# maotian123/loc_lib

Measured on AMD Instinct MI355X. Metric: scans/sec (64x1800-pt scan vs 10M-pt map) + ICP iter ms, higher is better.
Workload: dtype f64; 1 GPU; BASELINE configs[2]: 256 scans/GPU x 115200 pts (64x1800, cityblock-v1) vs one 10000000-pt map, P2PLANE ICP, reference defaults (alpha=0.1 KD-tree ANN, eps=1e-2, max 20 iters), scans sharded by rank, no collective; includes scan H2D: every step aligns a batch copied host->HBM for it (pinned double buffer, copy stream, overlapped with the previous step); 3 alignment(s) in flight; scans_per_gpu=256, map_points=10000000, pipeline_depth=3, search_mode=tree_faithful_ann, tree_depth=30, tree_bytes=239999992

## Files before the change

### loc_lib_amd/api.py

```python
import ctypes
import os
import subprocess

import numpy as np

_HERE = os.path.dirname(os.path.abspath(__file__))
LIB_PATH = os.environ.get("LOCGPU_LIB") or os.path.join(_HERE, "liblocgpu.so")
CSRC = os.path.join(_HERE, "csrc")

P2P, P2LINE, P2PLANE = 0, 1, 2
P2PLANE_MAP = 5
SEARCH_TREE_FAITHFUL, SEARCH_GRID_EXACT = 0, 1
CENTER, NEARBY6 = 0, 1
DIRECT_NDT, INCREMENTAL_NDT = 1, 2

ABI_SYMBOLS = [
    "locgpu_icp_opts_default", "locgpu_ndt_opts_default", "locgpu_create", "locgpu_destroy", "locgpu_last_error",
    "locgpu_device_count", "locgpu_icp_set_target", "locgpu_icp_set_target_async", "locgpu_icp_target_info", "locgpu_knn", "locgpu_icp_hb", "locgpu_icp_align",
    "locgpu_transform_cloud", "locgpu_batch_create", "locgpu_batch_destroy", "locgpu_icp_align_batch", "locgpu_ndt_align_batch",
    "locgpu_icp_hb_batch", "locgpu_gn_update", "locgpu_ndt_set_target", "locgpu_ndt_target_info", "locgpu_ndt_dump",
    "locgpu_ndt_align", "locgpu_profile_enable", "locgpu_profile_read", "locgpu_visit_count_enable", "locgpu_visit_count_read",
    "locgpu_search_stats_read", "locgpu_debug_batch_nn", "locgpu_graph_enable",
    "locgpu_cloud_create", "locgpu_cloud_destroy", "locgpu_cloud_upload", "locgpu_cloud_info", "locgpu_cloud_download", "locgpu_cloud_copy",
    "locgpu_cloud_remove_nan", "locgpu_cloud_voxel_filter", "locgpu_cloud_crop_box", "locgpu_cloud_transform", "locgpu_cloud_append",
# ... 591 lines not shown
        out = np.zeros(6)
        self._check(lib().locgpu_profile_read(self._h, out.ctypes.data, int(reset)))
        return dict(search_ms=out[0], accum_ms=out[1], solve_ms=out[2], search_n=int(out[3]), accum_n=int(out[4]), solve_n=int(out[5]))

    def visit_count_enable(self, on=True):
        self._check(lib().locgpu_visit_count_enable(self._h, int(on)))

    def visit_count_read(self, reset=True):
        out = np.zeros(4, dtype=np.uint64)
        self._check(lib().locgpu_visit_count_read(self._h, out.ctypes.data, int(reset)))
        return dict(nodes=int(out[0]), leaves=int(out[1]), queries=int(out[2]), distinct_slots=int(out[3]))


    def debug_batch_nn(self, batch, k=5):
        out = np.empty((batch.n_local, batch.max_points, k), dtype=np.int32)
        self._check(lib().locgpu_debug_batch_nn(self._h, batch._h, int(k), out.ctypes.data))
        return out

    def search_stats_read(self, reset=True):
        out = np.zeros(4, dtype=np.uint64)
        self._check(lib().locgpu_search_stats_read(self._h, out.ctypes.data, int(reset)))
        return dict(searched=int(out[0]), redone=int(out[1]), walked=int(out[2]), replayed=int(out[3]))


def _xyzi(a):
    a = np.ascontiguousarray(a, dtype=np.float32)
    if a.ndim != 2 or a.shape[1] != 4:
        raise ValueError("cloud must be [n, 4] float32 (x, y, z, intensity)")
    return a


class Cloud:

    def __init__(self, ctx, points=None, is_dense=True, _borrowed=None):
        self.ctx = ctx
        self._owned = _borrowed is None
        if _borrowed is not None:
            self._h = _borrowed
        else:
            self._h = ctypes.c_void_p()
            ctx._check(lib().locgpu_cloud_create(ctx._h, ctypes.byref(self._h)))
            if points is not None:
                self.upload(points, is_dense)

    def upload(self, points, is_dense=True):
        a = _xyzi(points)
# ... 429 lines not shown
```

### loc_lib_amd/csrc/context.hpp

```cpp
#pragma once
#include <hip/hip_runtime.h>

#include <string>
#include <vector>

#include "../../include/locgpu.h"
#include "batch_upload.hpp"
#include "device_math.hpp"
#include "grid_kernels.hpp"
#include "icp_kernels.hpp"

#include "host_worker.hpp"

struct NdtTable;
namespace locgpu { struct IncNdtState; struct FilterScratch; }

namespace locgpu {
struct PendingTarget;
struct AlignSpec {
    GnParams prm{};
    float alpha = 1.0f;
    bool grid = false;
    bool ndt() const { return method_is_ndt(prm.method); }
    int k() const { return method_k(prm.method); }
// ... 78 lines not shown
    int slot = 0;
    hipStream_t stream = nullptr;
    int n_scans = 0, max_n = 0, blocks_per_scan = 0;
    int n_total = 0, first = 0;
    bool sharded = false;
    double* d_acc = nullptr;
    size_t pitch = 0;
    float4* d_src = nullptr;
    int* d_counts = nullptr;
    locgpu::PoseState* d_state = nullptr;
    uint32_t* d_nn = nullptr;
    bool shared_src = false;
    int* d_src_of = nullptr;
    int cap_scans = 0, split_scans = 0;
    size_t cap_points = 0;
    const float4* d_src_ext = nullptr;
    bool counters_clean = false;
    int last_iterations = -1;
    double* d_partials = nullptr;
    double* d_hb = nullptr;
    uint32_t* d_redo_list = nullptr;
    unsigned int* d_redo_count = nullptr;
    uint32_t* d_redo_list2 = nullptr;
    uint32_t* d_grid_qkey = nullptr;
    uint2* d_grid_sorted = nullptr;
    uint32_t* d_grid_tile_count = nullptr;
    void* d_grid_scan_temp = nullptr;
    size_t grid_tocc_cap = 0, grid_scan_cap = 0;
    hipGraphExec_t graph_exec = nullptr;
    hipGraphExec_t graph_exec_next = nullptr;
    locgpu::AlignSpec graph_spec;
    const void* graph_target = nullptr;
    unsigned long long graph_epoch = 0;
    float4* h_src = nullptr;
    hipEvent_t xyz_ev[8] = {};
    locgpu::PoseState* h_state = nullptr;
    unsigned long long* h_post = nullptr;
    static constexpr int kPostWord = 16;
    unsigned int post_call = 0;
    bool paced_tail = false;
    hipEvent_t tail_ev = nullptr;
    double* h_hb = nullptr;
    int* h_active = nullptr;
    int* d_active = nullptr;
    std::vector<int> counts;
    locgpu::BatchUploadState upl;
// ... 39 lines not shown
```

### loc_lib_amd/csrc/gn_driver.hip

```cpp
#include <algorithm>
#include <chrono>
#include <cmath>
#include <cstdlib>
#include <cstring>
#include <string>
#include <thread>

#include "batch_upload.hpp"
#include "env.hpp"
#include "gn_driver.hpp"
#include "ndt_inc.hpp"
#include "ndt_kernels.hpp"

namespace locgpu {

namespace {
inline int next_chunk(const locgpu_batch* b) { return b->n_total == 1 ? 2 : kNextChunk; }
inline int first_chunk_len(const locgpu_batch* b) {
    if (b->n_total != 1 || b->sharded || b->last_iterations < 0) return kFirstChunk;
    return std::min(kLongFirstChunk, std::max(3, b->last_iterations + 1));
}

}

SearchArgs make_search_args(const locgpu_ctx* ctx, const locgpu_batch* b, const float4* src, const PoseState* st, int k, float alpha_eff, bool skip_nonfinite) {
    SearchArgs sa{ctx->d_tree, ctx->tree_slots * sizeof(uint64_t), ctx->depth, src, b->d_counts, st, b->d_nn, b->pitch, b->max_n, b->n_scans, k, alpha_eff,
                  skip_nonfinite ? 1 : 0, nullptr, b->d_redo_list, b->d_redo_count, b->d_redo_list2, b->d_redo_count + 1, ctx->d_search_stats};
    if (!ctx->tree_bounded) sa.redo_list = nullptr;
    return sa;
}

void init_state(PoseState& ps, const double pose[7]) {
    std::memset(&ps, 0, sizeof(ps));
    for (int i = 0; i < 4; ++i) ps.q[i] = pose[i];
    for (int i = 0; i < 3; ++i) ps.t[i] = pose[4 + i];
    quat_to_R(ps.q, ps.R);
}

static void init_states(locgpu_batch* b, const double* poses) {
    for (int s = 0; s < b->n_total; ++s) init_state(b->h_state[s], poses + 7 * (size_t)s);
}

void write_scan_result(const PoseState& ps, const double* init, double* out_pose, locgpu_align_stats* stats) {
    if (ps.status == 1) {
        for (int j = 0; j < 7; ++j) out_pose[j] = init[j];
    } else {
        for (int j = 0; j < 4; ++j) out_pose[j] = ps.q[j];
        for (int j = 0; j < 3; ++j) out_pose[4 + j] = ps.t[j];
    }
    if (!stats) return;
// ... 494 lines not shown
```

### loc_lib_amd/csrc/icp_search.hip

```cpp
#include "env.hpp"
#include "icp_kernels.hpp"
#include "launch.hpp"
#include "search_walk.hpp"

#include <algorithm>
#include <iterator>
#include <type_traits>
#include <utility>

namespace locgpu {

template <int KMAX, int D, bool COUNT>
__global__ __launch_bounds__(kBlock) void icp_search_kernel(const uint2* __restrict__ tree, const float4* __restrict__ src,
                                                            const int* __restrict__ counts, const PoseState* __restrict__ st,
                                                            uint32_t* __restrict__ nn, size_t nn_pitch, int max_n, int k, float alpha_eff,
                                                            int skip_nonfinite, unsigned long long* __restrict__ visit_totals, uint32_t* __restrict__ touched,
                                                            const int* __restrict__ active, const int* __restrict__ src_of) {
    __shared__ uint32_t s_far[D][kBlock];
    __shared__ float s_d2[D][kBlock];
    const int scan = active ? active[blockIdx.y] : (int)blockIdx.y;
    if (st[scan].done) return;
    const int tid = threadIdx.x;
    const int i = blockIdx.x * kBlock + tid;
    if (i >= counts[scan]) return;
// ... 149 lines not shown
    for (unsigned int r0 = blockIdx.x * per_wave; r0 < n; r0 += gridDim.x * per_wave) {
        const unsigned int r = r0 + (unsigned int)tid;
        const bool valid = (unsigned int)tid < per_wave && r < n;
        const uint32_t gi = valid ? list[r] : 0u;
        Walk<K> w;
        w.qx = w.qy = w.qz = 0.f;
        if (valid) {
            int scan;
            const float4 p = list_point(src, src_of, max_n, gi, scan);
            const D3 qs = se3_apply(st[scan].q, st[scan].t, D3{(double)p.x, (double)p.y, (double)p.z});
            w.qx = (float)qs.x; w.qy = (float)qs.y; w.qz = (float)qs.z;
        }
        walk_query<K, ROWB>(rsrc, tree, w, valid, alpha_eff, 0, dummy, (uint32_t)(size_t)(&s_dyn[tid]), 0x7fffffff);
        const bool slow = valid && w.slow != 0u;
        if (valid && !slow) {
#pragma unroll
            for (int j = 0; j < K; ++j) nn[(size_t)j * nn_pitch + gi] = w.id[j];
        }
        if (!walk_exact_in_wave<K>(tree, slow, w.qx, w.qy, w.qz, alpha_eff, s_dyn, nn, nn_pitch, gi, search_stats))
            wave_append(redo_list, redo_count, slow, gi);
    }
}

constexpr int kRedoWaves = 2048;
constexpr int kDeepLanes = 64, kDeepWaves = 2048;
template <int KMAX, int D>
__global__ __launch_bounds__(64) void icp_search_redo_kernel(const uint2* __restrict__ tree, const float4* __restrict__ src,
                                                             const PoseState* __restrict__ st, uint32_t* __restrict__ nn, size_t nn_pitch,
                                                             int max_n, int k, float alpha_eff, const uint32_t* __restrict__ redo_list,
                                                             const unsigned int* __restrict__ redo_count, unsigned long long* __restrict__ search_stats,
                                                             const int* __restrict__ src_of) {
    __shared__ uint32_t s_far[D][64];
    __shared__ float s_d2[D][64];
    const unsigned int n = *redo_count;
    const int tid = threadIdx.x;
    if (blockIdx.x == 0 && tid == 0 && search_stats) atomicAdd(&search_stats[1], (unsigned long long)n);
    const unsigned int per_wave = min(64u, (n + gridDim.x - 1) / gridDim.x);
    if ((unsigned)tid >= per_wave) return;
    for (unsigned int r = blockIdx.x * per_wave + tid; r < n; r += gridDim.x * per_wave) {
        const size_t gi = redo_list[r];
        int scan;
        const float4 p = list_point(src, src_of, max_n, gi, scan);
        const D3 qs = se3_apply(st[scan].q, st[scan].t, D3{(double)p.x, (double)p.y, (double)p.z});
        KnnHeap<KMAX> heap;
        uint32_t nvis = 0, lvis = 0, out[KMAX];
        int cnt;
// ... 17 lines not shown
    KnnHeap<KMAX> heap;
    uint32_t nvis = 0, lvis = 0;
    tree_knn<KMAX, D, true>(tree, queries[3 * i], queries[3 * i + 1], queries[3 * i + 2], k, alpha_eff, s_far, s_d2, tid, heap, nvis, lvis);
    uint32_t out[KMAX];
    int cnt;
    heap_to_sorted<KMAX>(heap, out, cnt);
#pragma unroll
    for (int j = 0; j < KMAX; ++j)
        if (j < k) out_idx[i * k + j] = (out[j] == kInvalidSlot) ? -1 : (int32_t)(tree[out[j]].y & 0x3FFFFFFFu);
    if (visits) { visits[2 * i] = nvis; visits[2 * i + 1] = lvis; }
}

__global__ __launch_bounds__(kBlock) void count_touched_kernel(uint32_t* __restrict__ touched, size_t n_words, unsigned long long* __restrict__ totals) {
    unsigned long long c = 0;
    for (size_t i = (size_t)blockIdx.x * kBlock + threadIdx.x; i < n_words; i += (size_t)gridDim.x * kBlock) {
        c += (unsigned long long)__popc(touched[i]);
        touched[i] = 0u;
    }
    for (int off = 32; off > 0; off >>= 1) c += __shfl_xor(c, off, 64);
    if ((threadIdx.x & 63) == 0 && c) atomicAdd(&totals[3], c);
}

__global__ __launch_bounds__(kBlock) void nn_to_index_kernel(const uint2* __restrict__ tree, const uint32_t* __restrict__ nn, size_t nn_pitch, size_t n_queries,
                                                             int k, int32_t* __restrict__ out) {
    const size_t gi = (size_t)blockIdx.x * kBlock + threadIdx.x;
    if (gi >= n_queries) return;
    for (int j = 0; j < k; ++j) {
        const uint32_t slot = nn[(size_t)j * nn_pitch + gi];
        out[gi * k + j] = slot == kInvalidSlot ? -1 : (int32_t)(tree[slot].y & 0x3FFFFFFFu);
    }
}


template <class F>
static bool with_depth(int depth, F&& f) {
    if (depth <= 32) f(std::integral_constant<int, 32>{});
    else if (depth <= 40) f(std::integral_constant<int, 40>{});
    else if (depth <= 64) f(std::integral_constant<int, 64>{});
    else return false;
    return true;
}
template <bool UP_TO, class F>
static bool with_k(int k, F&& f) {
    if (k == 1) return f(std::integral_constant<int, 1>{});
    if (UP_TO ? k <= 5 : k == 5) return f(std::integral_constant<int, 5>{});
    if constexpr (UP_TO)
        if (k <= 8) return f(std::integral_constant<int, 8>{});
    return false;
}

bool stamp_build() {
    static const bool on = env_int("LOCGPU_STAMP", 0) != 0;
    return on;
}

void launch_nn_to_index(const uint2* tree, const uint32_t* nn, size_t nn_pitch, size_t n_queries, int k, int32_t* out, hipStream_t s) {
    hipLaunchKernelGGL(nn_to_index_kernel, dim3((unsigned)((n_queries + kBlock - 1) / kBlock)), dim3(kBlock), 0, s, tree, nn, nn_pitch, n_queries, k, out);
}

void launch_count_touched(uint32_t* touched, size_t n_words, unsigned long long* totals, hipStream_t s) {
    hipLaunchKernelGGL(count_touched_kernel, dim3(1024), dim3(kBlock), 0, s, touched, n_words, totals);
}

template <int KMAX, int D, bool COUNT>
static void launch_exact(const SearchArgs& a, hipStream_t s) {
    dim3 grid((a.max_n + kBlock - 1) / kBlock, a.active ? a.n_active : a.n_scans);
    hipLaunchKernelGGL((icp_search_kernel<KMAX, D, COUNT>), grid, dim3(kBlock), 0, s, a.tree, a.src, a.counts, a.st, a.nn, a.nn_pitch, a.max_n,
                       a.k, a.alpha_eff, a.skip_nonfinite, a.visit_totals, COUNT ? a.touched : nullptr, a.active, a.src_of);
}

struct WalkShape { int df, win; };
constexpr WalkShape kWalkShapes[] = {{10, 8}, {12, 0}, {15, 0}, {24, 0}};
template <class F, size_t... I>
static bool all_walk_shapes(F&& f, std::index_sequence<I...>) {
    return (f(std::integral_constant<int, kWalkShapes[I].df>{}, std::integral_constant<int, kWalkShapes[I].win>{}) && ...);
}
template <class F>
static bool all_walk_shapes(F&& f) { return all_walk_shapes(f, std::make_index_sequence<std::size(kWalkShapes)>{}); }

static int fast_stack_depth() {
    static const int v = [] {
        const int e = env_int("LOCGPU_FAST_STACK", kWalkShapes[0].df);
        for (const WalkShape& w : kWalkShapes)
            if (w.df == e) return e;
        return kWalkShapes[0].df;
    }();
    return v;
}
constexpr int kWindowStored = 13;

template <auto Kernel>
static bool no_static_lds() {
    hipFuncAttributes attr{};
    return hipFuncGetAttributes(&attr, reinterpret_cast<const void*>(Kernel)) == hipSuccess && attr.sharedSizeBytes == 0;
}
template <int K>
static bool walk_kernels_ok() {
    bool ok = all_walk_shapes([](auto DF, auto WIN) {
        return no_static_lds<icp_search_walk_kernel<K, DF(), 64, false, WIN()>>() && no_static_lds<icp_search_walk_kernel<K, DF(), 64, true, WIN()>>();
    });
    for (int depth : {32, 40, 64})
        with_depth(depth, [&](auto D) { ok = ok && no_static_lds<icp_search_walk_kernel<K, D() + 2, 16>>() && no_static_lds<icp_search_walk_list_kernel<K, D(), kDeepLanes>>(); });
    return ok;
}
bool search_kernels_lds_ok() {
    static const bool ok = walk_kernels_ok<1>() && walk_kernels_ok<5>();
    return ok;
}

template <int K, int D>
static void launch_redo(const SearchArgs& a, hipStream_t s) {
    hipLaunchKernelGGL((icp_search_redo_kernel<K, D>), dim3(kRedoWaves), dim3(64), 0, s, a.tree, a.src, a.st, a.nn, a.nn_pitch, a.max_n, a.k,
                       a.alpha_eff, a.redo_list, a.redo_count, a.search_stats, a.src_of);
}
template <int K, int D>
static void launch_walk_list(const SearchArgs& a, const uint32_t* list, const unsigned int* n_list, hipStream_t s) {
    hipLaunchKernelGGL((icp_search_walk_list_kernel<K, D, kDeepLanes>), dim3(kDeepWaves), dim3(64), (D + 2) * kDeepLanes * 8, s, a.tree, a.src, a.st, a.nn, a.nn_pitch, a.max_n,
                       a.alpha_eff, (unsigned int)a.tree_bytes + 16u, (uint32_t)(a.tree_bytes / 8), list, n_list, a.redo_list, a.redo_count, a.search_stats, a.src_of);
}

template <int K, int D, int DF, int WIN>
static void launch_walk(const SearchArgs& a, hipStream_t s) {
    const bool stamp = stamp_build();
    const uint32_t dummy = (uint32_t)(a.tree_bytes / 8);
    const unsigned int rsrc_bytes = (unsigned int)a.tree_bytes + 16u;
    const int n_launch = a.active ? a.n_active : a.n_scans;
    if (!stamp && (size_t)((a.max_n + 63) / 64) * n_launch <= 2048) {
        dim3 g1((a.max_n + 15) / 16, n_launch);
        hipLaunchKernelGGL((icp_search_walk_kernel<K, D + 2, 16>), g1, dim3(64), (D + 2) * 16 * 8, s, a.tree, a.src, a.counts, a.st, a.nn, a.nn_pitch, a.max_n,
                           a.alpha_eff, 0, rsrc_bytes, dummy, a.skip_nonfinite, a.redo_list, a.redo_count, a.redo_list2, a.redo_count2, a.search_stats, a.active, a.src_of);
        return;
    }
    const int stored = WIN ? kWindowStored : DF - 2;
    const int Tw = a.depth > stored ? a.depth - stored : 0;
    dim3 g2((a.max_n + 63) / 64, n_launch);
    static const bool lds_knob = env_flag("LOCGPU_K1_LDS_BYTES");
    unsigned lds_bytes = DF * 64 * 8;
    if (lds_knob) lds_bytes = (unsigned)std::max(env_int("LOCGPU_K1_LDS_BYTES", 0), DF * 64 * 8);
    if (stamp)
// ... 52 lines not shown
```

### loc_lib_amd/csrc/launch.hpp

```cpp
#pragma once
#include "gn_post.hpp"
#include <hip/hip_runtime.h>
#include <stdint.h>

#include "device_math.hpp"

namespace locgpu {

struct GnParams;

struct SearchArgs {
    const uint2* tree;
    size_t tree_bytes;
    int depth;
    const float4* src;
    const int* counts;
    const PoseState* st;
    uint32_t* nn;
    size_t nn_pitch;
    int max_n, n_scans, k;
    float alpha_eff;
    int skip_nonfinite;
    unsigned long long* visit_totals;
    uint32_t* redo_list;
    unsigned int* redo_count;
    uint32_t* redo_list2;
    unsigned int* redo_count2;
    unsigned long long* search_stats;
    const int* active = nullptr;
    int n_active = 0;
    const int* src_of = nullptr;
    uint32_t* touched = nullptr;
};

struct AccumArgs {
    const uint2* tree;
    const float4* src;
    const int* counts;
    const PoseState* st;
    const uint32_t* nn;
    size_t nn_pitch;
    int max_n, n_scans;
    double gate;
    double* partials;
    const int* active = nullptr;
    int n_active = 0;
    const int* src_of = nullptr;
    int split_scans = 0;
    const double* planes = nullptr;
};

bool launch_icp_search(const SearchArgs& a, hipStream_t s);
bool launch_icp_search_redo(const SearchArgs& a, hipStream_t s);
bool launch_icp_search_list(const SearchArgs& a, const uint32_t* list, const unsigned int* n_list, hipStream_t s);
bool launch_knn_query(const uint2* tree, int depth, const float* q, size_t nq, int k, float alpha_eff, int32_t* out, uint32_t* visits,
                      hipStream_t s);
// ... 27 lines not shown
    int max_n, n_scans;
    float gate2;
    double* partials;
    double* out;
    unsigned int* list_counts;
    const int* src_of = nullptr;
};
int icp_fitness_rows(int max_n);
void launch_icp_fitness(const FitnessArgs& a, hipStream_t s);
int launch_icp_fitness_accum(const FitnessArgs& a, hipStream_t s);
void launch_loam_fitness_sum(const double* const partials[2], const int rows[2], int n_cands, double* out, unsigned int* const list_counts[2], hipStream_t s);
void launch_fitness_sum(const double* partials, int rows, int n_scans, double* out, unsigned int* list_counts, hipStream_t s);
struct M12f { float v[12]; };
void launch_transform_cloud(const float4* src, size_t n, const M12f& m12, float* dst_xyz, hipStream_t s);
void launch_loam_join_transform(const float4* edge, size_t n_edge, const float4* surf, size_t n_surf, const M12f& m12, float4* out, hipStream_t s);
void launch_map_plane_queries(const uint2* tree, const uint32_t* leaf_slots, size_t first, int n, float4* src, int* counts, hipStream_t s);
void launch_map_plane_fit(const uint2* tree, const uint32_t* leaf_slots, size_t first, int n, const uint32_t* nn, size_t nn_pitch, double* planes,
                          unsigned long long* n_valid, hipStream_t s);
void launch_map_plane_dump(const uint2* tree, const uint32_t* leaf_slots, size_t n_leaves, const double* planes, size_t n_points, double* out_n4,
                           unsigned char* out_valid, hipStream_t s);
bool search_kernels_lds_ok();
bool stamp_build();
void launch_count_touched(uint32_t* touched, size_t n_words, unsigned long long* totals, hipStream_t s);
void launch_nn_to_index(const uint2* tree, const uint32_t* nn, size_t nn_pitch, size_t n_queries, int k, int32_t* out, hipStream_t s);

}
```

### loc_lib_amd/csrc/locgpu_api.hip

```cpp
#include <algorithm>
#include <atomic>
#include <cmath>
#include <cstdio>
#include <cstdlib>
#include <cstring>
#include <string>
#include <vector>

#include "batch_upload.hpp"
#include "cloud_filters.hpp"
#include "context.hpp"
#include "gn_driver.hpp"
#include "launch.hpp"
#include "ndt_inc.hpp"
#include "ndt_kernels.hpp"
#include "search_chunks.hpp"

using namespace locgpu;

namespace {
std::string g_create_err;
}

namespace locgpu {
// ... 10 lines not shown
}

static bool fill_now(locgpu_ctx* ctx, void* p, size_t bytes, const char* what) {
    return hip_ok(ctx, hipMemsetAsync(p, 0, bytes, ctx->stream), what) && hip_ok(ctx, hipStreamSynchronize(ctx->stream), what);
}

void locgpu::free_batch(locgpu_batch* b) {
    if (!b) return;
    upload_free_batch(b);
    for (hipEvent_t ev : b->stage_ev.ev) (void)hipEventDestroy(ev);
    if (b->ev_ready) (void)hipEventDestroy(b->ev_ready);
    if (b->ev_reduced) (void)hipEventDestroy(b->ev_reduced);
    if (b->d_src) (void)hipFree(b->d_src);
    if (b->d_src_of) (void)hipFree(b->d_src_of);
    if (b->d_counts) (void)hipFree(b->d_counts);
    if (b->d_state) (void)hipFree(b->d_state);
    if (b->d_nn) (void)hipFree(b->d_nn);
    if (b->d_partials) (void)hipFree(b->d_partials);
    if (b->d_hb) (void)hipFree(b->d_hb);
    if (b->d_acc) (void)hipFree(b->d_acc);
    if (b->d_redo_list) (void)hipFree(b->d_redo_list);
    if (b->d_redo_count) (void)hipFree(b->d_redo_count);
    if (b->d_redo_list2) (void)hipFree(b->d_redo_list2);
    if (b->d_grid_qkey) (void)hipFree(b->d_grid_qkey);
    if (b->d_grid_sorted) (void)hipFree(b->d_grid_sorted);
    if (b->d_grid_tile_count) (void)hipFree(b->d_grid_tile_count);
    if (b->d_grid_scan_temp) (void)hipFree(b->d_grid_scan_temp);
    if (b->graph_exec) (void)hipGraphExecDestroy(b->graph_exec);
    if (b->graph_exec_next) (void)hipGraphExecDestroy(b->graph_exec_next);
    if (b->h_src) (void)hipHostFree(b->h_src);
    if (b->h_state) (void)hipHostFree(b->h_state);
    if (b->h_post) (void)hipHostFree(b->h_post);
    if (b->tail_ev) (void)hipEventDestroy(b->tail_ev);
    for (hipEvent_t e : b->xyz_ev)
        if (e) (void)hipEventDestroy(e);
    if (b->h_hb) (void)hipHostFree(b->h_hb);
    if (b->h_active) (void)hipHostFree(b->h_active);
    if (b->d_active) (void)hipFree(b->d_active);
    delete b;
}

extern "C" {

void locgpu_icp_opts_default(locgpu_icp_opts* o) {
    if (!o) return;
    o->method = LOCGPU_P2P;
// ... 165 lines not shown
    if (n_scans < 0 || (n_scans == 0 && !sharded) || first < 0 || first + n_scans > n_total) return fail(ctx, LOCGPU_ERR_INVALID, "batch_create: bad arguments");
    if (n_total > 65535) return fail(ctx, LOCGPU_ERR_INVALID, "batch_create: at most 65535 scans per batch");
    if (n_scans > 65535) return fail(ctx, LOCGPU_ERR_INVALID, "batch_create: at most 65535 scans per batch");
    LOCGPU_HIP(ctx, hipSetDevice(ctx->device));
    if (n_scans == 0) max_n = 1;
    if (max_n == 0 || max_n > 0x7FFFFF00u || (size_t)n_scans * max_n > 0xFFFFFFF0ull)
        return fail(ctx, LOCGPU_ERR_INVALID, "batch_create: scans are empty or the batch exceeds 2^32 points");
    auto* b = new locgpu_batch();
    b->ctx = ctx;
    b->slot = ctx->next_slot;
    ctx->next_slot = (ctx->next_slot + 1) % locgpu_ctx::kSlots;
    b->stream = ctx->slot_stream[b->slot];
    b->n_scans = n_scans;
    b->n_total = n_total;
    b->first = first;
    b->sharded = sharded;
    b->max_n = (int)max_n;
    b->blocks_per_scan = (int)((max_n + kBlock - 1) / kBlock);
    b->pitch = (size_t)n_scans * max_n;
    b->counts.assign(n_scans, 0);
    b->shared_src = shared_src;
    b->cap_scans = n_scans;
    b->cap_points = max_n;
    bool ok = hip_ok(ctx, hipMalloc((void**)&b->d_src, std::max<size_t>(shared_src ? max_n : b->pitch, 1) * sizeof(float4)), "hipMalloc src") &&
              (!shared_src || (hip_ok(ctx, hipMalloc((void**)&b->d_src_of, (size_t)n_scans * sizeof(int)), "hipMalloc src_of") &&
                               fill_now(ctx, b->d_src_of, (size_t)n_scans * sizeof(int), "hipMemset src_of"))) &&
              hip_ok(ctx, hipMalloc((void**)&b->d_counts, std::max(n_scans, 1) * sizeof(int)), "hipMalloc counts") &&
              hip_ok(ctx, hipMalloc((void**)&b->d_state, n_total * sizeof(PoseState)), "hipMalloc state") &&
              (!sharded || hip_ok(ctx, hipMalloc((void**)&b->d_acc, (size_t)kFirstChunk * n_total * kAccW * sizeof(double)), "hipMalloc acc")) &&
              hip_ok(ctx, hipMalloc((void**)&b->d_nn, 5 * std::max<size_t>(b->pitch, 1) * sizeof(uint32_t)), "hipMalloc nn") &&
              hip_ok(ctx, hipMalloc((void**)&b->d_partials, (size_t)std::max(n_scans, 1) * b->blocks_per_scan * kAccW * sizeof(double)), "hipMalloc partials") &&
              hip_ok(ctx, hipMalloc((void**)&b->d_hb, (size_t)n_total * 44 * sizeof(double)), "hipMalloc hb") &&
              hip_ok(ctx, hipMalloc((void**)&b->d_redo_list, (stamp_build() ? 2 : 1) * std::max<size_t>(b->pitch, 1) * sizeof(uint32_t)), "hipMalloc redo") &&
              hip_ok(ctx, hipMalloc((void**)&b->d_redo_list2, std::max<size_t>(b->pitch, 1) * sizeof(uint32_t)), "hipMalloc redo2") &&
              hip_ok(ctx, hipMalloc((void**)&b->d_redo_count, 4 * sizeof(unsigned int)), "hipMalloc redo") &&
              hip_ok(ctx, hipHostMalloc((void**)&b->h_state, n_total * sizeof(PoseState)), "hipHostMalloc state") &&
              hip_ok(ctx, hipHostMalloc((void**)&b->h_hb, (size_t)n_total * 44 * sizeof(double)), "hipHostMalloc hb") &&
              hip_ok(ctx, hipHostMalloc((void**)&b->h_active, (size_t)std::max(n_scans, 1) * sizeof(int)), "hipHostMalloc active") &&
              hip_ok(ctx, hipMalloc((void**)&b->d_active, (size_t)std::max(n_scans, 1) * sizeof(int)), "hipMalloc active") &&
              fill_now(ctx, b->d_counts, std::max(n_scans, 1) * sizeof(int), "hipMemset counts") &&
              fill_now(ctx, b->d_redo_count, 4 * sizeof(unsigned int), "hipMemset redo");
    if (!ok) { free_batch(b); return LOCGPU_ERR_OOM; }
    *out = b;
    return LOCGPU_OK;
}

extern "C" {

static int make_batch(locgpu_ctx* ctx, const void* const* srcs, const size_t* counts, size_t stride_bytes, int n_scans, locgpu_batch** out,
                      int first = 0, int n_total = -1) {
    if (!ctx || !out) return LOCGPU_ERR_INVALID;
    *out = nullptr;
    if (n_scans < 0 || (n_scans > 0 && (!srcs || !counts)) || stride_bytes < 12) return fail(ctx, LOCGPU_ERR_INVALID, "batch_create: bad arguments");
    size_t max_n = 0;
    for (int s = 0; s < n_scans; ++s) max_n = std::max(max_n, counts[s]);
    for (int s = 0; s < n_scans; ++s)
        if (!srcs[s] && counts[s]) return fail(ctx, LOCGPU_ERR_INVALID, "batch_create: NULL scan pointer");
    locgpu_batch* b = nullptr;
// ... 182 lines not shown

int locgpu_icp_align(locgpu_ctx* ctx, const void* src, size_t n, size_t stride_bytes, const double init_pose[7], const locgpu_icp_opts* opts,
                     double out_pose[7], locgpu_align_stats* stats) {
    AlignSpec spec;
    const int rc = check_icp(ctx, opts, spec);
    return rc != LOCGPU_OK ? rc : align_single(ctx, spec, "icp_align", src && init_pose && out_pose, src, n, stride_bytes, nullptr, init_pose, out_pose, stats);
}

int locgpu_icp_hb_batch(locgpu_ctx* ctx, locgpu_batch* b, const double* poses, const locgpu_icp_opts* opts, double* hb) {
    AlignSpec spec;
    int rc = check_icp(ctx, opts, spec);
    if (rc == LOCGPU_OK) rc = check_batch(ctx, b, poses && hb, spec, "icp_hb_batch");
    return rc != LOCGPU_OK ? rc : eval_hb_batch(ctx, b, poses, spec, hb, "icp_hb_batch");
}

int locgpu_debug_batch_nn(locgpu_ctx* ctx, locgpu_batch* b, int k, int32_t* out) {
    if (!ctx || !b || b->ctx != ctx || !out || k < 1 || k > 5) return fail(ctx, LOCGPU_ERR_INVALID, "debug_batch_nn: bad arguments");
    { const int jrc = target_join(ctx); if (jrc != LOCGPU_OK) return jrc; }
    if (!ctx->d_tree) return fail(ctx, LOCGPU_ERR_NO_TARGET, "debug_batch_nn: no ICP target");
    LOCGPU_HIP(ctx, hipSetDevice(ctx->device));
    const size_t nq = (size_t)b->n_scans * b->max_n;
    int32_t* d_out = nullptr;
    LOCGPU_HIP(ctx, hipMalloc((void**)&d_out, nq * k * sizeof(int32_t)));
    launch_nn_to_index(ctx->d_tree, b->d_nn, b->pitch, nq, k, d_out, b->stream);
    const hipError_t e = hipMemcpyAsync(out, d_out, nq * k * sizeof(int32_t), hipMemcpyDeviceToHost, b->stream);
    const hipError_t e2 = hipStreamSynchronize(b->stream);
    (void)hipFree(d_out);
    LOCGPU_HIP(ctx, e);
    LOCGPU_HIP(ctx, e2);
    return LOCGPU_OK;
}

int locgpu_icp_hb(locgpu_ctx* ctx, const void* src, size_t n, size_t stride_bytes, const double pose[7], const locgpu_icp_opts* opts, double H[36],
                  double B[6], int64_t* effective_num, int* ok) {
    AlignSpec spec;
    int rc = check_icp(ctx, opts, spec);
    if (rc != LOCGPU_OK) return rc;
    if (!src || !pose || !H || !B) return fail(ctx, LOCGPU_ERR_INVALID, "icp_hb: bad arguments");
    locgpu_batch* b = nullptr;
    rc = single_batch(ctx, src, n, stride_bytes, &b);
    if (rc != LOCGPU_OK) return rc;
    double hb[44];
    rc = eval_hb_batch(ctx, b, pose, spec, hb, "icp_hb");
    if (rc != LOCGPU_OK) return rc;
    std::memcpy(H, hb, 36 * sizeof(double));
    std::memcpy(B, hb + 36, 6 * sizeof(double));
    if (effective_num) *effective_num = (int64_t)hb[42];
// ... 489 lines not shown
int locgpu_visit_count_read(locgpu_ctx* ctx, uint64_t out[4], int reset) {
    if (!ctx || !out) return LOCGPU_ERR_INVALID;
    out[0] = out[1] = out[2] = out[3] = 0;
    if (!ctx->d_visits) return LOCGPU_OK;
    LOCGPU_HIP(ctx, hipSetDevice(ctx->device));
    for (hipStream_t st : ctx->slot_stream) LOCGPU_HIP(ctx, hipStreamSynchronize(st));
    unsigned long long h[4];
    LOCGPU_HIP(ctx, hipMemcpy(h, ctx->d_visits, sizeof(h), hipMemcpyDeviceToHost));
    out[0] = h[0]; out[1] = h[1]; out[2] = h[2]; out[3] = h[3];
    if (reset && !fill_now(ctx, ctx->d_visits, sizeof(h), "hipMemset visits")) return LOCGPU_ERR_NO_DEVICE;
    return LOCGPU_OK;
}

}

extern "C" __attribute__((visibility("default"))) int locgpu_debug_stamp_trips(locgpu_ctx* ctx, locgpu_batch* b, uint32_t* out) {
    if (!ctx || !b || !out || !stamp_build()) return LOCGPU_ERR_INVALID;
    LOCGPU_HIP(ctx, hipSetDevice(ctx->device));
    LOCGPU_HIP(ctx, hipStreamSynchronize(b->stream));
    LOCGPU_HIP(ctx, hipMemcpy(out, b->d_redo_list + b->pitch, b->pitch * sizeof(uint32_t), hipMemcpyDeviceToHost));
    return LOCGPU_OK;
}

extern "C" __attribute__((visibility("default"))) size_t locgpu_debug_grid_dump(locgpu_ctx* ctx, int64_t info[9], float params[6], float* pts, size_t pts_cap,
                                                                                 void* tiles, size_t tiles_cap_bytes, uint32_t* hash, size_t hash_cap) {
    if (!ctx || target_join(ctx) != LOCGPU_OK || !ctx->d_tree || ensure_grid(ctx) != LOCGPU_OK) return 0;
    const locgpu::GridView& g = ctx->grid;
    if (info) {
        for (int a = 0; a < 3; ++a) { info[a] = g.dims[a]; info[6 + a] = g.tdims[a]; }
        info[3] = (int64_t)g.num_cells; info[4] = g.n_tocc; info[5] = (int64_t)g.tile_mask + 1;
    }
    if (params) { for (int a = 0; a < 3; ++a) params[a] = g.origin[a]; params[3] = g.cell; params[4] = g.inv_cell; params[5] = g.slack; }
    if (pts && hipMemcpy(pts, g.pts, std::min(pts_cap, g.num_points * 4) * sizeof(float), hipMemcpyDeviceToHost) != hipSuccess) return 0;
    if (tiles && hipMemcpy(tiles, g.tiles, std::min(tiles_cap_bytes, (size_t)g.n_tocc * sizeof(locgpu::TileRec)), hipMemcpyDeviceToHost) != hipSuccess) return 0;
    if (hash && hipMemcpy(hash, g.tile_hash, std::min(hash_cap, ((size_t)g.tile_mask + 1) * 2) * sizeof(uint32_t), hipMemcpyDeviceToHost) != hipSuccess) return 0;
    return g.num_points;
}

namespace locgpu {
void ndt_free(locgpu_ctx* ctx) {
    if (ctx->ndt) { ndt_table_free(*ctx->ndt); delete ctx->ndt; ctx->ndt = nullptr; }
    if (ctx->inc) { inc_ndt_destroy(ctx->inc); ctx->inc = nullptr; }
}
int check_ndt(locgpu_ctx* ctx, AlignSpec& spec) {
    if (!ctx) return LOCGPU_ERR_INVALID;
    const bool inc = ctx->ndt_opts.method == kNdtOptIncremental;
// ... 168 lines not shown
```

### loc_lib_amd/csrc/search_walk.hpp

```cpp
#pragma once
#include "icp_kernels.hpp"

namespace locgpu {

constexpr float kSentinelCoord = 3.0e38f;

template <int K>
struct Walk {
    float qx, qy, qz;
    float d[K];
    uint32_t id[K];
    uint32_t cur;
    int avail;
    uint32_t c3n;
    uint32_t slow;
    uint32_t rounds, wave_rounds;
};

typedef uint32_t __attribute__((address_space(3))) lds_u32;
typedef uint32_t u32x2 __attribute__((ext_vector_type(2)));
typedef u32x2 __attribute__((address_space(3))) lds_u32x2;

__device__ __forceinline__ lds_u32* lds_ptr(uint32_t byte_addr) { return reinterpret_cast<lds_u32*>(byte_addr); }

// ... 205 lines not shown
        for (int step = 0; step < C; ++step) {
            if (n.y < 0xC0000000u) {
                const uint32_t meta = n.y;
                const float th = as_f32(n.x);
                const float qa = meta < 0x40000000u ? qx : (meta < 0x80000000u ? qy : qz);
                const float dd = qa - th;
                const uint32_t nd2 = __float_as_uint(-(dd * dd));
                const uint32_t right = meta & 0x3FFFFFFFu;
                const bool go_left = qa < th;
                const uint32_t cur1 = cur + 1u;
                *reinterpret_cast<lds_u32x2*>(col_addr + (uint32_t)avail * ROWB) = u32x2{go_left ? right : cur1, nd2};
                avail += (int)nd2 < nbound ? 1 : 0;
                cur = go_left ? cur1 : right;
                n = __builtin_amdgcn_raw_buffer_load_b128(rsrc, (int)(cur << 3), 0, 0);
            }
        }
    } while (__ballot(cur != dummy || avail > 0) != 0ull);
#pragma unroll
    for (int j = 0; j < K; ++j) { w.d[j] = d[j]; w.id[j] = id[j]; }
    w.slow = slow; w.c3n = c3n; w.cur = cur; w.avail = avail;
    if (STAMP) { w.rounds = my_rounds; w.wave_rounds = all_rounds; }
}

}
```

Measured before the change: 12090 scans/s.

## Add spill-to-global ring-buffer stack for deep KD-tree list walks

Adds a new deep-query search kernel whose traversal stack is a small LDS ring window (default 8 rows) that spills older entries to a per-wave global buffer and reloads them in chunks when needed. This replaces the deep-list kernel that reserved a full depth-sized LDS stack per lane. The smaller LDS footprint allows higher occupancy, with waves_per_eu pinned at 8. The cost is extra global traffic and divergence on spill and reload, plus a fallback to the slow path when the spill rows overflow. It also masks nn_to_index output for padded query slots and adds a debug stats entry point.

```diff
diff --git a/loc_lib_amd/api.py b/loc_lib_amd/api.py
--- a/loc_lib_amd/api.py
+++ b/loc_lib_amd/api.py
@@ -637,6 +637,13 @@
         self._check(lib().locgpu_search_stats_read(self._h, out.ctypes.data, int(reset)))
         return dict(searched=int(out[0]), redone=int(out[1]), walked=int(out[2]), replayed=int(out[3]))
 
+    def debug_deep_stats(self):
+        fn = lib().locgpu_debug_deep_stats
+        fn.restype, fn.argtypes = ctypes.c_int, [ctypes.c_void_p, ctypes.c_void_p]
+        out = np.zeros(3, dtype=np.uint64)
+        self._check(fn(self._h, out.ctypes.data))
+        return dict(deep=int(out[0]), spilled=int(out[1]), reloaded=int(out[2]))
+
 
 def _xyzi(a):
     a = np.ascontiguousarray(a, dtype=np.float32)
diff --git a/loc_lib_amd/csrc/context.hpp b/loc_lib_amd/csrc/context.hpp
--- a/loc_lib_amd/csrc/context.hpp
+++ b/loc_lib_amd/csrc/context.hpp
@@ -124,6 +124,8 @@
     uint32_t* d_redo_list = nullptr;
     unsigned int* d_redo_count = nullptr;
     uint32_t* d_redo_list2 = nullptr;
+    uint2* d_deep_spill = nullptr;
+    int deep_spill_waves = 0;
     uint32_t* d_grid_qkey = nullptr;
     uint2* d_grid_sorted = nullptr;
     uint32_t* d_grid_tile_count = nullptr;
diff --git a/loc_lib_amd/csrc/gn_driver.hip b/loc_lib_amd/csrc/gn_driver.hip
--- a/loc_lib_amd/csrc/gn_driver.hip
+++ b/loc_lib_amd/csrc/gn_driver.hip
@@ -26,6 +26,7 @@
 SearchArgs make_search_args(const locgpu_ctx* ctx, const locgpu_batch* b, const float4* src, const PoseState* st, int k, float alpha_eff, bool skip_nonfinite) {
     SearchArgs sa{ctx->d_tree, ctx->tree_slots * sizeof(uint64_t), ctx->depth, src, b->d_counts, st, b->d_nn, b->pitch, b->max_n, b->n_scans, k, alpha_eff,
                   skip_nonfinite ? 1 : 0, nullptr, b->d_redo_list, b->d_redo_count, b->d_redo_list2, b->d_redo_count + 1, ctx->d_search_stats};
+    sa.deep_spill = b->d_deep_spill; sa.deep_spill_waves = b->deep_spill_waves;
     if (!ctx->tree_bounded) sa.redo_list = nullptr;
     return sa;
 }
diff --git a/loc_lib_amd/csrc/icp_search.hip b/loc_lib_amd/csrc/icp_search.hip
--- a/loc_lib_amd/csrc/icp_search.hip
+++ b/loc_lib_amd/csrc/icp_search.hip
@@ -195,6 +195,55 @@
     }
 }
 
+template <int K, int WIN, bool STAMP = false>
+__global__ __launch_bounds__(64) __attribute__((amdgpu_waves_per_eu(8, 8))) void icp_search_walk_spill_kernel(const uint2* __restrict__ tree, const float4* __restrict__ src,
+                                                                   const PoseState* __restrict__ st, uint32_t* __restrict__ nn, size_t nn_pitch, int max_n,
+                                                                   float alpha_eff, unsigned int tree_bytes, uint32_t dummy, const uint32_t* __restrict__ list,
+                                                                   const unsigned int* __restrict__ n_list, uint32_t* __restrict__ redo_list,
+                                                                   unsigned int* __restrict__ redo_count, unsigned long long* __restrict__ search_stats,
+                                                                   const int* __restrict__ src_of, uint2* __restrict__ spill, int spill_rows) {
+    extern __shared__ uint2 s_dyn[];
+    static_assert(WIN * 64 * 8 >= 64 * 2 * 8, "exact stack columns do not fit");
+    const unsigned int n = *n_list;
+    const int tid = threadIdx.x;
+    if (blockIdx.x == 0 && tid == 0 && search_stats) atomicAdd(&search_stats[2], (unsigned long long)n);
+    const __amdgpu_buffer_rsrc_t rsrc = __builtin_amdgcn_make_buffer_rsrc((void*)tree, 0, (int)tree_bytes, 0x00020000);
+    u32x2* spill_col = reinterpret_cast<u32x2*>(spill) + (size_t)blockIdx.x * (size_t)spill_rows * 64 + tid;
+    const unsigned int per_wave = min(64u, max(1u, (n + gridDim.x - 1) / gridDim.x));
+    for (unsigned int r0 = blockIdx.x * per_wave; r0 < n; r0 += gridDim.x * per_wave) {
+        const unsigned int r = r0 + (unsigned int)tid;
+        const bool valid = (unsigned int)tid < per_wave && r < n;
+        const uint32_t gi = valid ? list[r] : 0u;
+        Walk<K> w;
+        w.qx = w.qy = w.qz = 0.f;
+        if (valid) {
+            int scan;
+            const float4 p = list_point(src, src_of, max_n, gi, scan);
+            const D3 qs = se3_apply(st[scan].q, st[scan].t, D3{(double)p.x, (double)p.y, (double)p.z});
+            w.qx = (float)qs.x; w.qy = (float)qs.y; w.qz = (float)qs.z;
+        }
+#pragma unroll
+        for (int j = 0; j < K; ++j) { w.d[j] = __builtin_inff(); w.id[j] = kInvalidSlot; }
+        const bool sane = fabsf(w.qx) < 1e18f && fabsf(w.qy) < 1e18f && fabsf(w.qz) < 1e18f;
+        w.slow = valid && !sane ? 1u : 0u;
+        uint32_t n_spilled = 0, n_reloaded = 0;
+        walk_spill<K, WIN, LOCGPU_K1_C, STAMP>(rsrc, w, valid && sane, alpha_eff, dummy, (uint32_t)(size_t)(&s_dyn[tid]), spill_col, spill_rows, n_spilled, n_reloaded);
+#pragma unroll
+        for (int j = 0; j + 1 < K; ++j) w.slow |= w.d[j] == w.d[j + 1] ? 1u : 0u;
+        if (STAMP && search_stats && valid) {
+            if (n_spilled) atomicAdd(&search_stats[5], (unsigned long long)n_spilled);
+            if (n_reloaded) atomicAdd(&search_stats[6], (unsigned long long)n_reloaded);
+        }
+        const bool slow = valid && w.slow != 0u;
+        if (valid && !slow) {
+#pragma unroll
+            for (int j = 0; j < K; ++j) nn[(size_t)j * nn_pitch + gi] = w.id[j];
+        }
+        if (!walk_exact_in_wave<K>(tree, slow, w.qx, w.qy, w.qz, alpha_eff, s_dyn, nn, nn_pitch, gi, search_stats))
+            wave_append(redo_list, redo_count, slow, gi);
+    }
+}
+
 constexpr int kRedoWaves = 2048;
 constexpr int kDeepLanes = 64, kDeepWaves = 2048;
 template <int KMAX, int D>
@@ -258,11 +307,12 @@
 }
 
 __global__ __launch_bounds__(kBlock) void nn_to_index_kernel(const uint2* __restrict__ tree, const uint32_t* __restrict__ nn, size_t nn_pitch, size_t n_queries,
-                                                             int k, int32_t* __restrict__ out) {
+                                                             int k, int32_t* __restrict__ out, const int* __restrict__ counts, int max_n) {
     const size_t gi = (size_t)blockIdx.x * kBlock + threadIdx.x;
     if (gi >= n_queries) return;
+    const bool searched = (int)(gi % (size_t)max_n) < counts[gi / (size_t)max_n];
     for (int j = 0; j < k; ++j) {
-        const uint32_t slot = nn[(size_t)j * nn_pitch + gi];
+        const uint32_t slot = searched ? nn[(size_t)j * nn_pitch + gi] : kInvalidSlot;
         out[gi * k + j] = slot == kInvalidSlot ? -1 : (int32_t)(tree[slot].y & 0x3FFFFFFFu);
     }
 }
@@ -290,8 +340,8 @@
     return on;
 }
 
-void launch_nn_to_index(const uint2* tree, const uint32_t* nn, size_t nn_pitch, size_t n_queries, int k, int32_t* out, hipStream_t s) {
-    hipLaunchKernelGGL(nn_to_index_kernel, dim3((unsigned)((n_queries + kBlock - 1) / kBlock)), dim3(kBlock), 0, s, tree, nn, nn_pitch, n_queries, k, out);
+void launch_nn_to_index(const uint2* tree, const uint32_t* nn, size_t nn_pitch, size_t n_queries, int k, int32_t* out, const int* counts, int max_n, hipStream_t s) {
+    hipLaunchKernelGGL(nn_to_index_kernel, dim3((unsigned)((n_queries + kBlock - 1) / kBlock)), dim3(kBlock), 0, s, tree, nn, nn_pitch, n_queries, k, out, counts, max_n);
 }
 
 void launch_count_touched(uint32_t* touched, size_t n_words, unsigned long long* totals, hipStream_t s) {
@@ -325,6 +375,24 @@
 }
 constexpr int kWindowStored = 13;
 
+constexpr int kDeepWindows[] = {8, 2, 4, 6, 12};
+template <class F, size_t... I>
+static bool all_deep_windows(F&& f, std::index_sequence<I...>) { return (f(std::integral_constant<int, kDeepWindows[I]>{}) && ...); }
+template <class F>
+static bool all_deep_windows(F&& f) { return all_deep_windows(f, std::make_index_sequence<std::size(kDeepWindows)>{}); }
+
+int deep_window() {
+    static const int v = [] {
+        const int e = env_int("LOCGPU_DEEP_WIN", kDeepWindows[0]);
+        if (e == 0) return 0;
+        for (int w : kDeepWindows)
+            if (w == e) return e;
+        return kDeepWindows[0];
+    }();
+    return v;
+}
+int deep_spill_waves(size_t pitch) { return (int)std::min<size_t>(kDeepSpillWaves, std::max<size_t>((pitch + 15) / 16, 1)); }
+
 template <auto Kernel>
 static bool no_static_lds() {
     hipFuncAttributes attr{};
@@ -337,7 +405,9 @@
     });
     for (int depth : {32, 40, 64})
         with_depth(depth, [&](auto D) { ok = ok && no_static_lds<icp_search_walk_kernel<K, D() + 2, 16>>() && no_static_lds<icp_search_walk_list_kernel<K, D(), kDeepLanes>>(); });
-    return ok;
+    return ok && all_deep_windows([](auto WIN) {
+               return no_static_lds<icp_search_walk_spill_kernel<K, WIN(), false>>() && no_static_lds<icp_search_walk_spill_kernel<K, WIN(), true>>();
+           });
 }
 bool search_kernels_lds_ok() {
     static const bool ok = walk_kernels_ok<1>() && walk_kernels_ok<5>();
@@ -351,6 +421,23 @@
 }
 template <int K, int D>
 static void launch_walk_list(const SearchArgs& a, const uint32_t* list, const unsigned int* n_list, hipStream_t s) {
+    const int win = a.deep_spill ? deep_window() : 0;
+    if (win != 0) {
+        const bool stamp = stamp_build();
+        const unsigned waves = (unsigned)std::min(a.deep_spill_waves, deep_spill_waves(a.nn_pitch));
+        all_deep_windows([&](auto WIN) {
+            if (WIN() != win) return true;
+            auto launch = [&](auto kernel) {
+                hipLaunchKernelGGL(kernel, dim3(waves), dim3(64), WIN() * 64 * 8, s, a.tree, a.src, a.st, a.nn, a.nn_pitch, a.max_n, a.alpha_eff,
+                                   (unsigned int)a.tree_bytes + 16u, (uint32_t)(a.tree_bytes / 8), list, n_list, a.redo_list, a.redo_count, a.search_stats, a.src_of,
+                                   a.deep_spill, kDeepSpillRows);
+            };
+            if (stamp) launch(icp_search_walk_spill_kernel<K, WIN(), true>);
+            else launch(icp_search_walk_spill_kernel<K, WIN(), false>);
+            return false;
+        });
+        return;
+    }
     hipLaunchKernelGGL((icp_search_walk_list_kernel<K, D, kDeepLanes>), dim3(kDeepWaves), dim3(64), (D + 2) * kDeepLanes * 8, s, a.tree, a.src, a.st, a.nn, a.nn_pitch, a.max_n,
                        a.alpha_eff, (unsigned int)a.tree_bytes + 16u, (uint32_t)(a.tree_bytes / 8), list, n_list, a.redo_list, a.redo_count, a.search_stats, a.src_of);
 }
diff --git a/loc_lib_amd/csrc/launch.hpp b/loc_lib_amd/csrc/launch.hpp
--- a/loc_lib_amd/csrc/launch.hpp
+++ b/loc_lib_amd/csrc/launch.hpp
@@ -31,7 +31,13 @@
     int n_active = 0;
     const int* src_of = nullptr;
     uint32_t* touched = nullptr;
+    uint2* deep_spill = nullptr;
+    int deep_spill_waves = 0;
 };
+
+constexpr int kDeepSpillRows = 32, kDeepSpillWaves = 8192;
+int deep_window();
+int deep_spill_waves(size_t pitch);
 
 struct AccumArgs {
     const uint2* tree;
@@ -105,6 +111,6 @@
 bool search_kernels_lds_ok();
 bool stamp_build();
 void launch_count_touched(uint32_t* touched, size_t n_words, unsigned long long* totals, hipStream_t s);
-void launch_nn_to_index(const uint2* tree, const uint32_t* nn, size_t nn_pitch, size_t n_queries, int k, int32_t* out, hipStream_t s);
+void launch_nn_to_index(const uint2* tree, const uint32_t* nn, size_t nn_pitch, size_t n_queries, int k, int32_t* out, const int* counts, int max_n, hipStream_t s);
 
 }
diff --git a/loc_lib_amd/csrc/locgpu_api.hip b/loc_lib_amd/csrc/locgpu_api.hip
--- a/loc_lib_amd/csrc/locgpu_api.hip
+++ b/loc_lib_amd/csrc/locgpu_api.hip
@@ -56,6 +56,7 @@
     if (b->d_redo_list) (void)hipFree(b->d_redo_list);
     if (b->d_redo_count) (void)hipFree(b->d_redo_count);
     if (b->d_redo_list2) (void)hipFree(b->d_redo_list2);
+    if (b->d_deep_spill) (void)hipFree(b->d_deep_spill);
     if (b->d_grid_qkey) (void)hipFree(b->d_grid_qkey);
     if (b->d_grid_sorted) (void)hipFree(b->d_grid_sorted);
     if (b->d_grid_tile_count) (void)hipFree(b->d_grid_tile_count);
@@ -267,6 +268,7 @@
     b->shared_src = shared_src;
     b->cap_scans = n_scans;
     b->cap_points = max_n;
+    b->deep_spill_waves = deep_window() != 0 ? deep_spill_waves(b->pitch) : 0;
     bool ok = hip_ok(ctx, hipMalloc((void**)&b->d_src, std::max<size_t>(shared_src ? max_n : b->pitch, 1) * sizeof(float4)), "hipMalloc src") &&
               (!shared_src || (hip_ok(ctx, hipMalloc((void**)&b->d_src_of, (size_t)n_scans * sizeof(int)), "hipMalloc src_of") &&
                                fill_now(ctx, b->d_src_of, (size_t)n_scans * sizeof(int), "hipMemset src_of"))) &&
@@ -279,6 +281,8 @@
               hip_ok(ctx, hipMalloc((void**)&b->d_redo_list, (stamp_build() ? 2 : 1) * std::max<size_t>(b->pitch, 1) * sizeof(uint32_t)), "hipMalloc redo") &&
               hip_ok(ctx, hipMalloc((void**)&b->d_redo_list2, std::max<size_t>(b->pitch, 1) * sizeof(uint32_t)), "hipMalloc redo2") &&
               hip_ok(ctx, hipMalloc((void**)&b->d_redo_count, 4 * sizeof(unsigned int)), "hipMalloc redo") &&
+              (b->deep_spill_waves == 0 ||
+               hip_ok(ctx, hipMalloc((void**)&b->d_deep_spill, (size_t)b->deep_spill_waves * kDeepSpillRows * 64 * sizeof(uint2)), "hipMalloc deep spill")) &&
               hip_ok(ctx, hipHostMalloc((void**)&b->h_state, n_total * sizeof(PoseState)), "hipHostMalloc state") &&
               hip_ok(ctx, hipHostMalloc((void**)&b->h_hb, (size_t)n_total * 44 * sizeof(double)), "hipHostMalloc hb") &&
               hip_ok(ctx, hipHostMalloc((void**)&b->h_active, (size_t)std::max(n_scans, 1) * sizeof(int)), "hipHostMalloc active") &&
@@ -507,7 +511,7 @@
     const size_t nq = (size_t)b->n_scans * b->max_n;
     int32_t* d_out = nullptr;
     LOCGPU_HIP(ctx, hipMalloc((void**)&d_out, nq * k * sizeof(int32_t)));
-    launch_nn_to_index(ctx->d_tree, b->d_nn, b->pitch, nq, k, d_out, b->stream);
+    launch_nn_to_index(ctx->d_tree, b->d_nn, b->pitch, nq, k, d_out, b->d_counts, b->max_n, b->stream);
     const hipError_t e = hipMemcpyAsync(out, d_out, nq * k * sizeof(int32_t), hipMemcpyDeviceToHost, b->stream);
     const hipError_t e2 = hipStreamSynchronize(b->stream);
     (void)hipFree(d_out);
@@ -1043,6 +1047,16 @@
     return LOCGPU_OK;
 }
 
+extern "C" __attribute__((visibility("default"))) int locgpu_debug_deep_stats(locgpu_ctx* ctx, uint64_t out[3]) {
+    if (!ctx || !out || !stamp_build() || !ctx->d_search_stats) return LOCGPU_ERR_INVALID;
+    LOCGPU_HIP(ctx, hipSetDevice(ctx->device));
+    for (hipStream_t st : ctx->slot_stream) LOCGPU_HIP(ctx, hipStreamSynchronize(st));
+    unsigned long long h[7];
+    LOCGPU_HIP(ctx, hipMemcpy(h, ctx->d_search_stats, sizeof(h), hipMemcpyDeviceToHost));
+    out[0] = h[2]; out[1] = h[5]; out[2] = h[6];
+    return LOCGPU_OK;
+}
+
 extern "C" __attribute__((visibility("default"))) size_t locgpu_debug_grid_dump(locgpu_ctx* ctx, int64_t info[9], float params[6], float* pts, size_t pts_cap,
                                                                                  void* tiles, size_t tiles_cap_bytes, uint32_t* hash, size_t hash_cap) {
     if (!ctx || target_join(ctx) != LOCGPU_OK || !ctx->d_tree || ensure_grid(ctx) != LOCGPU_OK) return 0;
diff --git a/loc_lib_amd/csrc/search_walk.hpp b/loc_lib_amd/csrc/search_walk.hpp
--- a/loc_lib_amd/csrc/search_walk.hpp
+++ b/loc_lib_amd/csrc/search_walk.hpp
@@ -251,4 +251,134 @@
     if (STAMP) { w.rounds = my_rounds; w.wave_rounds = all_rounds; }
 }
 
-}
+template <int WIN>
+__device__ __forceinline__ uint32_t ring_row(int logical) {
+    if constexpr ((WIN & (WIN - 1)) == 0) return (uint32_t)logical & (uint32_t)(WIN - 1);
+    else return (uint32_t)(logical + 4 * WIN) % (uint32_t)WIN;
+}
+
+template <int K, int WIN, int C, bool STAMP = false>
+__device__ __forceinline__ void walk_spill(__amdgpu_buffer_rsrc_t rsrc, Walk<K>& w, bool active, float alpha, uint32_t dummy, uint32_t col_addr,
+                                           u32x2* __restrict__ spill_col, int spill_rows, uint32_t& n_spilled, uint32_t& n_reloaded) {
+    constexpr uint32_t ROWB = 64 * 8;
+    constexpr int RELOAD = WIN < 4 ? WIN : 4;
+    static_assert(WIN >= 2 && (((WIN & (WIN - 1)) == 0) || WIN >= 4), "ring_row's offset covers four rows below the bottom");
+    const float qx = w.qx, qy = w.qy, qz = w.qz;
+    uint32_t cur = active ? 0u : dummy;
+    int avail = 0, base = 0;
+    float d[K];
+    uint32_t id[K];
+#pragma unroll
+    for (int j = 0; j < K; ++j) { d[j] = w.d[j]; id[j] = w.id[j]; }
+    uint32_t slow = w.slow;
+    auto step = [&](const u32x4& n, bool keep_all, int nbound) {
+        const uint32_t meta = n.y;
+        const float th = as_f32(n.x);
+        const float qa = meta < 0x40000000u ? qx : (meta < 0x80000000u ? qy : qz);
+        const float dd = qa - th;
+        const uint32_t nd2 = __float_as_uint(-(dd * dd));
+        const uint32_t right = meta & 0x3FFFFFFFu;
+        const bool go_left = qa < th;
+        const uint32_t cur1 = cur + 1u;
+        bool keep = keep_all || (int)nd2 < nbound;
+        const uint32_t slot = col_addr + ring_row<WIN>(avail) * ROWB;
+        cur = go_left ? cur1 : right;
+        const bool full = keep && avail - base == WIN;
+        if (__ballot(full) != 0ull) {
+            if (full) {
+                if (base < spill_rows) {
+                    __builtin_nontemporal_store(*reinterpret_cast<lds_u32x2*>(slot), &spill_col[(size_t)base * 64]);
+                    base++;
+                    if (STAMP) n_spilled++;
+                } else {
+                    slow = 1u; cur = dummy; avail = 0; base = 0; keep = false;
+                }
+            }
+        }
+        if (keep) {
+            *reinterpret_cast<lds_u32x2*>(slot) = u32x2{go_left ? right : cur1, nd2};
+            avail++;
+        }
+    };
+    u32x4 n = __builtin_amdgcn_raw_buffer_load_b128(rsrc, (int)(cur << 3), 0, 0);
+    while (__ballot(n.y < 0xC0000000u) != 0ull) {
+        if (n.y < 0xC0000000u) {
+            step(n, true, 0);
+            n = __builtin_amdgcn_raw_buffer_load_b128(rsrc, (int)(cur << 3), 0, 0);
+        }
+    }
+    do {
+        const bool is_leaf = n.y >= 0xC0000000u;
+        const bool need = is_leaf && avail == base && base > 0;
+        if (__ballot(need) != 0ull) {
+            if (need) {
+                const int cnt = base < RELOAD ? base : RELOAD;
+#pragma unroll
+                for (int j = 1; j <= RELOAD; ++j) {
+                    if (j <= cnt) {
+                        const u32x2 v = __builtin_nontemporal_load(&spill_col[(size_t)(base - j) * 64]);
+                        *reinterpret_cast<lds_u32x2*>(col_addr + ring_row<WIN>(base - j) * ROWB) = v;
+                    }
+                }
+                base -= cnt;
+                if (STAMP) n_reloaded += (uint32_t)cnt;
+            }
+        }
+        const u32x2 r0 = *reinterpret_cast<lds_u32x2*>(col_addr + ring_row<WIN>(avail - 1) * ROWB),
+                    r1 = *reinterpret_cast<lds_u32x2*>(col_addr + ring_row<WIN>(avail - 2) * ROWB),
+                    r2 = *reinterpret_cast<lds_u32x2*>(col_addr + ring_row<WIN>(avail - 3) * ROWB),
+                    r3 = *reinterpret_cast<lds_u32x2*>(col_addr + ring_row<WIN>(avail - 4) * ROWB);
+        const float dx = qx - as_f32(n.x), dy = qy - as_f32(n.z), dz = qz - as_f32(n.w);
+        const float dis2 = dx * dx + (dy * dy + dz * dz);
+        const float x = is_leaf ? dis2 : __builtin_inff();
+        bool c[K];
+#pragma unroll
+        for (int j = 0; j < K; ++j) c[j] = x < d[j];
+        if (K >= 2) {
+            const float gap = d[K - 1] - d[K - 2];
+            slow = ((gap == 0.0f) & c[K - 1]) ? 1u : slow;
+        }
+#pragma unroll
+        for (int j = K - 1; j >= 1; --j) {
+            const uint32_t below = id[j - 1], here = id[j];
+            const uint32_t t = c[j] ? cur : here;
+            id[j] = c[j - 1] ? below : t;
+            d[j] = __builtin_amdgcn_fmed3f(d[j - 1], x, d[j]);
+        }
+        {
+            const uint32_t here = id[0];
+            id[0] = c[0] ? cur : here;
+            d[0] = c[0] ? x : d[0];
+        }
+        const int nbound = (int)__float_as_uint(-(d[K - 1] * alpha));
+        const int nb = is_leaf ? nbound : (int)0x80000000u;
+        int hit = 4;
+        uint32_t nxt = cur;
+        hit = (int)r3.y < nb ? 3 : hit; nxt = (int)r3.y < nb ? r3.x : nxt;
+        hit = (int)r2.y < nb ? 2 : hit; nxt = (int)r2.y < nb ? r2.x : nxt;
+        hit = (int)r1.y < nb ? 1 : hit; nxt = (int)r1.y < nb ? r1.x : nxt;
+        hit = (int)r0.y < nb ? 0 : hit; nxt = (int)r0.y < nb ? r0.x : nxt;
+        const int held = is_leaf ? avail - base : 0;
+        const int m = held < 4 ? held : 4;
+        const bool ok = hit < m;
+        const uint32_t stay = is_leaf ? dummy : cur;
+        nxt = ok ? nxt : stay;
+        const int used = ok ? hit + 1 : m;
+        const bool moved = nxt != cur;
+        cur = nxt;
+        avail -= used;
+        if (moved) n = __builtin_amdgcn_raw_buffer_load_b128(rsrc, (int)(cur << 3), 0, 0);
+#pragma unroll
+        for (int s = 0; s < C; ++s) {
+            if (n.y < 0xC0000000u) {
+                step(n, false, nbound);
+                n = __builtin_amdgcn_raw_buffer_load_b128(rsrc, (int)(cur << 3), 0, 0);
+            }
+        }
+    } while (__ballot(cur != dummy || avail > 0) != 0ull);
+#pragma unroll
+    for (int j = 0; j < K; ++j) { w.d[j] = d[j]; w.id[j] = id[j]; }
+    w.slow = slow; w.cur = cur; w.avail = avail; w.c3n = 0u;
+}
+
+}
```

After: 11740 scans/s. 2.9% lower.
